# MengAiDev/SmokePhysAI

Measured on AMD Instinct MI355X. Metric: simulated+encoded frames/sec at 256^2 grid, batch 64, higher is better.
Workload: dtype f32 stencil + bf16x3 encoder (split-bf16 MFMA, fp32 accumulate)

## Files before the change

### smokephysai_amd/csrc/stencil.hip

```cpp
#include <map>
#include <mutex>

#include "stencil.h"

#include <math.h>
#include <stdlib.h>
#include <type_traits>

namespace smk {

#define TX 64
#define TY 4

__device__ __forceinline__ float clampf(float x, float lo, float hi) {
    float t = x < lo ? lo : x;
    return t > hi ? hi : t;
}
__device__ __forceinline__ int clampi(int x, int lo, int hi) {
    int t = x < lo ? lo : x;
    return t > hi ? hi : t;
}

__global__ void k_zero_state(Geom g, StateView s, const uint8_t *mask) {
    int b = blockIdx.z;
// ... 161 lines not shown
            float lap = v[(size_t)iu * g.pv + g.W] + v[(size_t)id * g.pv + g.W];
            lap = lap + vc.w;
            lap = lap + c;
            lap = lap - 4.0f * c;
            out.v[b * g.sv + (size_t)i * g.pv + g.W] = c + g.coef_uv * lap;
        }
    }
}

hipError_t launch_buoy_diffuse(const Geom &g, StateView in, StateView out, hipStream_t st) {
    if (g.W % 4 == 0 && g.pc % 4 == 0 && g.pv % 4 == 0) {
        dim3 grid(cdiv(g.W / 4, TX), cdiv(g.H + 1, TY), g.B), block(TX, TY);
        hipLaunchKernelGGL(k_buoy_diffuse4, grid, block, 0, st, g, in, out);
        return hipGetLastError();
    }
    dim3 grid(cdiv(g.W + 1, TX), cdiv(g.H + 1, TY), g.B), block(TX, TY);
    hipLaunchKernelGGL(k_buoy_diffuse, grid, block, 0, st, g, in, out);
    return hipGetLastError();
}

__global__ void k_divergence(Geom g, const float *u, const float *v, float *div, int dp, size_t ds) {
    int b = blockIdx.z;
    int j = blockIdx.x * TX + threadIdx.x, i = blockIdx.y * TY + threadIdx.y;
    if (i >= g.H || j >= g.W) return;
    const float *ub = u + b * g.su, *vb = v + b * g.sv;
    float a = ub[(size_t)(i + 1) * g.pc + j] - ub[(size_t)i * g.pc + j];
    a = a + vb[(size_t)i * g.pv + j + 1];
    a = a - vb[(size_t)i * g.pv + j];
    div[b * ds + (size_t)i * dp + j] = __fdiv_rn(a, g.dt);
}

hipError_t launch_divergence(const Geom &g, const float *u, const float *v, float *div, int dp, size_t ds,
                             hipStream_t st) {
    dim3 grid(cdiv(g.W, TX), cdiv(g.H, TY), g.B), block(TX, TY);
    hipLaunchKernelGGL(k_divergence, grid, block, 0, st, g, u, v, div, dp, ds);
    return hipGetLastError();
}

__global__ void k_jacobi_sweep(Geom g, const float *p, float *pn, const float *div) {
    int b = blockIdx.z;
    int j = blockIdx.x * TX + threadIdx.x, i = blockIdx.y * TY + threadIdx.y;
    if (i >= g.H || j >= g.W) return;
    const float *pb = p + b * g.sc;
    size_t o = (size_t)i * g.pc + j;
    float r = 0.f;
    if (i > 0 && i < g.H - 1 && j > 0 && j < g.W - 1) {
        float s = pb[o - g.pc] + pb[o + g.pc];
        s = s + pb[o - 1];
        s = s + pb[o + 1];
        s = s - div[b * g.sc + o];
        r = 0.25f * s;
    }
    pn[b * g.sc + o] = r;
}

__global__ void k_copy_cells(Geom g, const float *src, float *dst) {
    int j = blockIdx.x * TX + threadIdx.x, i = blockIdx.y * TY + threadIdx.y;
    if (i >= g.H || j >= g.W) return;
    size_t o = blockIdx.z * g.sc + (size_t)i * g.pc + j;
    dst[o] = src[o];
}

__device__ __forceinline__ float wave_shr1(float x) {
    return __builtin_bit_cast(float, __builtin_amdgcn_mov_dpp(__builtin_bit_cast(int, x), 0x138, 0xf, 0xf, true));
}
__device__ __forceinline__ float wave_shl1(float x) {
    return __builtin_bit_cast(float, __builtin_amdgcn_mov_dpp(__builtin_bit_cast(int, x), 0x130, 0xf, 0xf, true));
}

constexpr int JB_NW = 16;

template <int VEC> struct VecT;
template <> struct VecT<1> { using type = float; };
template <> struct VecT<2> { using type = float2; };
template <> struct VecT<4> { using type = float4; };
template <> struct VecT<8> { using type = float4; };
template <int VEC>
__device__ __forceinline__ void ldv(float (&dst)[VEC], const float *src) {
    using V = typename VecT<VEC>::type;
    constexpr int N = sizeof(V) / 4;
#pragma unroll
    for (int q = 0; q < VEC / N; ++q) {
        const V t = reinterpret_cast<const V *>(src)[q];
        const float *f = reinterpret_cast<const float *>(&t);
#pragma unroll
        for (int c = 0; c < N; ++c) dst[q * N + c] = f[c];
    }
}
template <int VEC>
__device__ __forceinline__ void stv(float *dst, const float (&src)[VEC]) {
    using V = typename VecT<VEC>::type;
    constexpr int N = sizeof(V) / 4;
#pragma unroll
    for (int q = 0; q < VEC / N; ++q) {
        V t;
        float *f = reinterpret_cast<float *>(&t);
#pragma unroll
        for (int c = 0; c < N; ++c) f[c] = src[q * N + c];
        reinterpret_cast<V *>(dst)[q] = t;
    }
}

struct JacobiSync {
    unsigned *flags;
    unsigned *status;
    float *x0, *x1;
    unsigned base;
    int chunks, nb, grid0, ngrids, abort_slot, fault;
    long long timeout_ticks;
    const float *u_in, *v_in, *d_in;
    float *d_out;
};

template <int VEC>
__device__ __forceinline__ void ldv_sc1(float (&dst)[VEC], __amdgpu_buffer_rsrc_t rs, unsigned byte_off) {
    typedef unsigned int u32x4 __attribute__((ext_vector_type(4)));
    typedef unsigned int u32x2 __attribute__((ext_vector_type(2)));
    if constexpr (VEC >= 4) {
#pragma unroll
        for (int q = 0; q < VEC / 4; ++q) {
            const u32x4 t = __builtin_amdgcn_raw_buffer_load_b128(rs, byte_off + 16 * q, 0, 16);
#pragma unroll
            for (int c = 0; c < 4; ++c) dst[4 * q + c] = __uint_as_float(t[c]);
        }
    } else if constexpr (VEC == 2) {
        const u32x2 t = __builtin_amdgcn_raw_buffer_load_b64(rs, byte_off, 0, 16);
        dst[0] = __uint_as_float(t[0]);
        dst[1] = __uint_as_float(t[1]);
    } else {
        dst[0] = __uint_as_float(__builtin_amdgcn_raw_buffer_load_b32(rs, byte_off, 0, 16));
    }
}
template <int VEC>
__device__ __forceinline__ void stv_sc1(__amdgpu_buffer_rsrc_t rs, unsigned byte_off, const float (&src)[VEC]) {
    typedef unsigned int u32x4 __attribute__((ext_vector_type(4)));
    typedef unsigned int u32x2 __attribute__((ext_vector_type(2)));
    if constexpr (VEC >= 4) {
#pragma unroll
        for (int q = 0; q < VEC / 4; ++q) {
            u32x4 t;
#pragma unroll
            for (int c = 0; c < 4; ++c) t[c] = __float_as_uint(src[4 * q + c]);
            __builtin_amdgcn_raw_buffer_store_b128(t, rs, byte_off + 16 * q, 0, 16);
        }
    } else if constexpr (VEC == 2) {
        u32x2 t;
        t[0] = __float_as_uint(src[0]);
        t[1] = __float_as_uint(src[1]);
        __builtin_amdgcn_raw_buffer_store_b64(t, rs, byte_off, 0, 16);
    } else {
        __builtin_amdgcn_raw_buffer_store_b32(__float_as_uint(src[0]), rs, byte_off, 0, 16);
    }
}

template <int VEC, int RPW, int MODE, bool PERSIST = false, bool FOLD = false>
__global__ __launch_bounds__(JB_NW * 64) void k_jacobi_band(Geom g, const float *__restrict__ p_in,
                                                            float *__restrict__ p_out, float *__restrict__ div,
                                                            float *__restrict__ u, float *__restrict__ v,
                                                            int iters, int BR, JacobiSync sy) {
    constexpr int TR = JB_NW * RPW, ROWF = 64 * VEC;
    __shared__ float edge[2][JB_NW][2][ROWF];
    __shared__ int handoff_failed;
    const int lane = threadIdx.x & 63, wave = threadIdx.x >> 6;
    int band_, grid_, nb_;
    if constexpr (PERSIST) {
        nb_ = sy.nb;
        const int id = blockIdx.x;
        if ((sy.ngrids & 7) == 0) {
            const int xcd = id & 7, slot = id >> 3;
            grid_ = (slot / nb_) * 8 + xcd;
            band_ = slot % nb_;
        } else {
            grid_ = id / nb_;
            band_ = id % nb_;
        }
        grid_ += sy.grid0;
    } else {
        band_ = blockIdx.x; grid_ = blockIdx.y; nb_ = gridDim.x;
    }
    const int band = band_, b = grid_, nb = nb_, halo = BR;
    const int e_rows = TR - halo, m_rows = TR - 2 * halo;
    const int own0 = band == 0 ? 0 : e_rows + (band - 1) * m_rows;
    int own1 = band == nb - 1 ? g.H : e_rows + band * m_rows;
    own1 = own1 < g.H ? own1 : g.H;
    int r0 = band == 0 ? 0 : (band == nb - 1 ? g.H - TR : own0 - halo);
    if (r0 > g.H - TR) r0 = g.H - TR;
    if (r0 < 0) r0 = 0;
    const int row0 = r0 + wave * RPW, j0 = lane * VEC;
    const size_t base = b * g.sc + (size_t)row0 * g.pc + j0;
    float pv[RPW][VEC], dv[RPW][VEC];
    const bool first_col = lane == 0, last_col = lane == 63;
    if constexpr (FOLD) {
        const float *ui = sy.u_in + b * g.su, *vi = sy.v_in + b * g.sv, *di = sy.d_in + b * g.sc;
        float *uo = u + b * g.su, *vo = v + b * g.sv, *dout = sy.d_out + b * g.sc;
        const int H = g.H, W = g.W;
        auto rowu = [&](int i, float (&x)[VEC]) {
            i = i < 0 ? 0 : (i > H ? H : i);
            ldv<VEC>(x, ui + (size_t)i * g.pc + j0);
        };
        auto rowdv = [&](int i, float (&dx)[VEC], float (&vx)[VEC], float &vW) {
            i = i < 0 ? 0 : (i > H - 1 ? H - 1 : i);
            ldv<VEC>(dx, di + (size_t)i * g.pc + j0);
            ldv<VEC>(vx, vi + (size_t)i * g.pv + j0);
            vW = vi[(size_t)i * g.pv + W];
#pragma unroll
            for (int c = 0; c < VEC; ++c) {
                const float bb = dx[c] * 0.1f;
                vx[c] = vx[c] + g.dt * bb;
            }
        };
        auto lap = [&](const float (&cc)[VEC], const float (&up)[VEC], const float (&dn)[VEC], float left, float right, float coef,
                       float (&o)[VEC]) {
#pragma unroll
            for (int c = 0; c < VEC; ++c) {
                float l = up[c] + dn[c];
                l = l + (c > 0 ? cc[c - 1] : left);
                l = l + (c < VEC - 1 ? cc[c + 1] : right);
                l = l - 4.0f * cc[c];
                o[c] = cc[c] + coef * l;
            }
        };
        float um[VEC], uc[VEC], un[VEC], dm[VEC], dc[VEC], dn[VEC], vm[VEC], vc[VEC], vn[VEC], vWm, vWc, vWn;
        rowu(row0 - 1, um);
        rowu(row0, uc);
        rowdv(row0 - 1, dm, vm, vWm);
        rowdv(row0, dc, vc, vWc);
        float u2prev[VEC], v2keep[VEC + 1];
#pragma unroll
        for (int k = 0; k <= RPW; ++k) {
            const int gi = row0 + k;
            rowu(gi + 1, un);
            float u2[VEC];
            {
                const float sl = wave_shr1(uc[VEC - 1]), sr = wave_shl1(uc[0]);
                lap(uc, um, un, first_col ? uc[0] : sl, last_col ? uc[VEC - 1] : sr, g.coef_uv, u2);
            }
            if ((gi >= own0 && gi < own1) || (gi == H && band == nb - 1)) stv<VEC>(uo + (size_t)gi * g.pc + j0, u2);
            if (k > 0) {
#pragma unroll
                for (int c = 0; c < VEC; ++c) {
                    float a = u2[c] - u2prev[c];
                    a = a + v2keep[c + 1];
                    a = a - v2keep[c];
                    dv[k - 1][c] = __fdiv_rn(a, g.dt);
                }
            }
#pragma unroll
            for (int c = 0; c < VEC; ++c) { u2prev[c] = u2[c]; um[c] = uc[c]; uc[c] = un[c]; }
            if (k < RPW) {
                rowdv(gi + 1, dn, vn, vWn);
                float d2[VEC], v2[VEC];
                {
                    const float sl = wave_shr1(dc[VEC - 1]), sr = wave_shl1(dc[0]);
                    lap(dc, dm, dn, first_col ? dc[0] : sl, last_col ? dc[VEC - 1] : sr, g.coef_d, d2);
                }
                {
                    const float sl = wave_shr1(vc[VEC - 1]), sr = wave_shl1(vc[0]);
                    lap(vc, vm, vn, first_col ? vc[0] : sl, last_col ? vWc : sr, g.coef_uv, v2);
                }
                float lw = vWm + vWn;
                lw = lw + vc[VEC - 1];
                lw = lw + vWc;
                lw = lw - 4.0f * vWc;
                const float v2W = vWc + g.coef_uv * lw;
                if (gi >= own0 && gi < own1) {
                    stv<VEC>(dout + (size_t)gi * g.pc + j0, d2);
                    stv<VEC>(vo + (size_t)gi * g.pv + j0, v2);
                    if (last_col) vo[(size_t)gi * g.pv + W] = v2W;
                }
                const float nx = wave_shl1(v2[0]);
#pragma unroll
                for (int c = 0; c < VEC; ++c) v2keep[c] = v2[c];
                v2keep[VEC] = last_col ? v2W : nx;
#pragma unroll
                for (int c = 0; c < VEC; ++c) { dm[c] = dc[c]; dc[c] = dn[c]; vm[c] = vc[c]; vc[c] = vn[c]; }
                vWm = vWc; vWc = vWn;
            }
        }
    }
#pragma unroll
    for (int k = 0; k < RPW; ++k)
#pragma unroll
        for (int c = 0; c < VEC; ++c) pv[k][c] = p_in[base + (size_t)k * g.pc + c];
    if constexpr (FOLD) {
    } else if (MODE & 1) {
        const float *ub = u + b * g.su + (size_t)row0 * g.pc + j0, *vb = v + b * g.sv + (size_t)row0 * g.pv + j0;
#pragma unroll
        for (int k = 0; k < RPW; ++k) {
            float vr[VEC + 1];
#pragma unroll
            for (int c = 0; c <= VEC; ++c) vr[c] = vb[(size_t)k * g.pv + c];
#pragma unroll
            for (int c = 0; c < VEC; ++c) {
                float a = ub[(size_t)(k + 1) * g.pc + c] - ub[(size_t)k * g.pc + c];
                a = a + vr[c + 1];
                a = a - vr[c];
                dv[k][c] = __fdiv_rn(a, g.dt);
            }
            const int gi = row0 + k;
            if (!PERSIST && gi >= own0 && gi < own1) {
#pragma unroll
                for (int c = 0; c < VEC; ++c) div[base + (size_t)k * g.pc + c] = dv[k][c];
            }
        }
    } else {
#pragma unroll
        for (int k = 0; k < RPW; ++k)
#pragma unroll
            for (int c = 0; c < VEC; ++c) dv[k][c] = div[base + (size_t)k * g.pc + c];
    }
    const int ring_k = __builtin_amdgcn_readfirstlane(row0 == 0 ? 0 : (row0 + RPW == g.H ? RPW - 1 : -1));
    auto sweep = [&](const float (&src)[RPW][VEC], float (&dst)[RPW][VEC], int par) {
#pragma unroll
        for (int c = 0; c < VEC; ++c) {
            edge[par][wave][0][j0 + c] = src[0][c];
            edge[par][wave][1][j0 + c] = src[RPW - 1][c];
        }
        __builtin_amdgcn_sched_barrier(0);
        auto row = [&](int k, const float (&up)[VEC], const float (&dn)[VEC]) {
            const float lin = wave_shr1(src[k][VEC - 1]), rin = wave_shl1(src[k][0]);
#pragma unroll
            for (int c = 0; c < VEC; ++c) {
                const float l = c > 0 ? src[k][c - 1] : lin;
                const float r = c < VEC - 1 ? src[k][c + 1] : rin;
                float sm = up[c] + dn[c];
                sm = sm + l;
                sm = sm + r;
                sm = sm - dv[k][c];
                dst[k][c] = 0.25f * sm;
            }
            dst[k][0] = first_col ? 0.f : dst[k][0];
            dst[k][VEC - 1] = last_col ? 0.f : dst[k][VEC - 1];
        };
#pragma unroll
        for (int k = 1; k < RPW - 1; ++k) row(k, src[k - 1], src[k + 1]);
        __builtin_amdgcn_sched_barrier(0);
        __syncthreads();
        const float *eu = &edge[par][wave > 0 ? wave - 1 : 0][1][j0];
        const float *ed = &edge[par][wave < JB_NW - 1 ? wave + 1 : JB_NW - 1][0][j0];
        float above[VEC], below[VEC];
#pragma unroll
        for (int c = 0; c < VEC; ++c) {
            above[c] = eu[c];
            below[c] = ed[c];
        }
        if (RPW == 1) {
            row(0, above, below);
        } else {
            row(0, above, src[1]);
            row(RPW - 1, src[RPW - 2], below);
        }
#pragma unroll
        for (int c = 0; c < VEC; ++c) {
            dst[0][c] = ring_k == 0 ? 0.f : dst[0][c];
            dst[RPW - 1][c] = ring_k == RPW - 1 ? 0.f : dst[RPW - 1][c];
        }
    };
    float pw[RPW][VEC];
    auto run = [&](int n) {
        int it = 0;
        for (; it + 2 <= n; it += 2) {
            sweep(pv, pw, 0);
            sweep(pw, pv, 1);
        }
        if (it < n) {
            sweep(pv, pw, 0);
#pragma unroll
            for (int k = 0; k < RPW; ++k)
#pragma unroll
                for (int c = 0; c < VEC; ++c) pv[k][c] = pw[k][c];
        }
    };
    if constexpr (!PERSIST) {
        run(iters);
    } else {
        const int me = b * nb + band;
        const unsigned row_off = (unsigned)(base * sizeof(float));
        const unsigned pitch_b = (unsigned)(g.pc * sizeof(float));
        const unsigned xbytes = (unsigned)((size_t)(sy.grid0 + sy.ngrids) * g.sc * sizeof(float));
        const __amdgpu_buffer_rsrc_t rx0 = __builtin_amdgcn_make_buffer_rsrc(sy.x0, 0, xbytes, 0x00020000);
        const __amdgpu_buffer_rsrc_t rx1 = __builtin_amdgcn_make_buffer_rsrc(sy.x1, 0, xbytes, 0x00020000);
        int done = 0;
        if (threadIdx.x == 0) handoff_failed = 0;
        for (int c = 0; c < sy.chunks; ++c) {
            const int n = (iters - done + (sy.chunks - c) - 1) / (sy.chunks - c);
            run(n);
            done += n;
            if (c == sy.chunks - 1) break;
            const __amdgpu_buffer_rsrc_t rx = (c & 1) ? rx1 : rx0;
#pragma unroll
            for (int k = 0; k < RPW; ++k) {
                const int gi = row0 + k;
                const bool pub = (band > 0 && gi >= own0 && gi < own0 + halo) || (band < nb - 1 && gi >= own1 - halo && gi < own1);
                if (pub) stv_sc1<VEC>(rx, row_off + k * pitch_b, pv[k]);
            }
            asm volatile("s_waitcnt vmcnt(0)" ::: "memory");
            __syncthreads();
            if (threadIdx.x == 0) {
                const unsigned tgt = sy.base + (unsigned)c + 1u;
                if (!(sy.fault && me == sy.grid0 * nb))
                    __hip_atomic_store(sy.flags + me, tgt, __ATOMIC_RELAXED, __HIP_MEMORY_SCOPE_AGENT);
                const long long t0 = wall_clock64();
                for (;;) {
                    const bool up = band == 0 ||
                        (int)(__hip_atomic_load(sy.flags + me - 1, __ATOMIC_RELAXED, __HIP_MEMORY_SCOPE_AGENT) - tgt) >= 0;
                    const bool dn = band == nb - 1 ||
                        (int)(__hip_atomic_load(sy.flags + me + 1, __ATOMIC_RELAXED, __HIP_MEMORY_SCOPE_AGENT) - tgt) >= 0;
                    if (up && dn) break;
                    if (__hip_atomic_load(sy.flags + sy.abort_slot, __ATOMIC_RELAXED, __HIP_MEMORY_SCOPE_AGENT) != 0u) {
                        handoff_failed = 1;
                        break;
                    }
                    if (wall_clock64() - t0 > sy.timeout_ticks) {
                        __hip_atomic_store(sy.flags + sy.abort_slot, 1u, __ATOMIC_RELAXED, __HIP_MEMORY_SCOPE_AGENT);
                        __hip_atomic_store(sy.status, 1u, __ATOMIC_RELAXED, __HIP_MEMORY_SCOPE_SYSTEM);
                        handoff_failed = 1;
                        break;
                    }
                    __builtin_amdgcn_s_sleep(2);
                }
            }
            __syncthreads();
#pragma unroll
            for (int k = 0; k < RPW; ++k) {
                const int gi = row0 + k;
                const bool need = (gi >= own0 - halo && gi < own0) || (gi >= own1 && gi < own1 + halo);
                if (need) ldv_sc1<VEC>(pv[k], rx, row_off + k * pitch_b);
            }
        }
        if (sy.chunks > 1 && handoff_failed) {
#pragma unroll
            for (int k = 0; k < RPW; ++k)
#pragma unroll
                for (int c = 0; c < VEC; ++c) pv[k][c] = __builtin_nanf("");
        }
    }
#pragma unroll
    for (int k = 0; k < RPW; ++k) {
        const int gi = row0 + k;
        if (gi >= own0 && gi < own1) {
#pragma unroll
            for (int c = 0; c < VEC; ++c) p_out[base + (size_t)k * g.pc + c] = pv[k][c];
        }
    }
    if (MODE & 2) {
        __syncthreads();
#pragma unroll
        for (int c = 0; c < VEC; ++c) edge[0][wave][1][j0 + c] = pv[RPW - 1][c];
        __syncthreads();
        float above[VEC];
#pragma unroll
        for (int c = 0; c < VEC; ++c) above[c] = edge[0][wave > 0 ? wave - 1 : 0][1][j0 + c];
        float *ub = u + b * g.su + (size_t)row0 * g.pc + j0, *vb = v + b * g.sv + (size_t)row0 * g.pv + j0;
#pragma unroll
        for (int k = 0; k < RPW; ++k) {
            const int gi = row0 + k;
            const float lin = wave_shr1(pv[k][VEC - 1]);
            if (gi >= own0 && gi < own1) {
                float un[VEC], vn[VEC];
                ldv<VEC>(un, ub + (size_t)k * g.pc);
                ldv<VEC>(vn, vb + (size_t)k * g.pv);
#pragma unroll
                for (int c = 0; c < VEC; ++c) {
                    if (gi >= 1) {
                        const float pu = k > 0 ? pv[k - 1][c] : above[c];
                        const float gr = pv[k][c] - pu;
                        un[c] = un[c] - g.dt * gr;
                    }
                    const float pl = c > 0 ? pv[k][c - 1] : lin;
                    const float gr = pv[k][c] - pl;
                    const float nv = vn[c] - g.dt * gr;
                    vn[c] = (c == 0 && first_col) ? vn[c] : nv;
                }
                if (gi >= 1) stv<VEC>(ub + (size_t)k * g.pc, un);
                stv<VEC>(vb + (size_t)k * g.pv, vn);
            }
        }
    }
}

struct StencilKnobs {
    bool persist, fault;
    StencilKnobs() {
        auto flag = [](const char *n, bool dflt) { const char *v = getenv(n); return v ? v[0] == '1' : dflt; };
        persist = flag("SMK_JACOBI_PERSIST", true);
        fault = flag("SMK_JACOBI_FAULT", false);
    }
};
static const StencilKnobs &knobs() {
    static const StencilKnobs k;
    return k;
}

struct JacobiPlan { int vec, rpw, br, nb, halo; };
static bool plan_jacobi(const Geom &g, JacobiPlan &pl, int iters = 100, bool persist = false) {
    if (g.W % 64 != 0 || g.W / 64 > 8 || (g.W / 64 & (g.W / 64 - 1)) || g.pc % 4 != 0) return false;
    pl.vec = g.W / 64;
    const int rpws[] = {2, 3, 4, 6, 8};
    double best = 1e30;
    bool ok = false;
    for (int rpw : rpws) {
        if (pl.vec * rpw > 32) continue;
        const int TR = JB_NW * rpw;
        if (TR > g.H) continue;
        for (int nb = 1; nb <= g.H / 8; ++nb) {
            int halo = nb == 1 ? 1 << 20 : (nb * TR - g.H) / (2 * nb - 2);
            if (nb == 1 && TR != g.H) continue;
            if (nb * TR < g.H || halo < 2) continue;
            if (nb > 1) {
                if (halo > 64) halo = 64;
                if (halo > (TR - 1) / 2) halo = (TR - 1) / 2;
                if ((TR - halo) + (nb - 2) * (TR - 2 * halo) >= g.H) continue;
            }
            if (persist && nb > 1) {
                const int e_rows = TR - halo, m_rows = TR - 2 * halo, last = g.H - (e_rows + (nb - 2) * m_rows);
                if (e_rows <= halo || last <= halo || (nb > 2 && m_rows <= halo) || nb > 64) continue;
            }
            const int br = halo;
            const double wgs = (double)nb * g.B, rounds = ceil(wgs / 256.0);
            const double cost_per_sweep = rounds * TR * (1.33 / 96.0), launch = 6.0;
            const double cost = persist ? launch + (ceil((double)iters / halo) - 1) * 3.5 + iters * cost_per_sweep
                                        : 2 * ceil(0.5 * iters / halo) * launch + iters * cost_per_sweep;
            if (cost < best) { best = cost; pl.rpw = rpw; pl.br = br; pl.nb = nb; pl.halo = halo; ok = true; }
        }
    }
    return ok;
}


template <int VEC, int MODE>
static void launch_band(const Geom &g, const JacobiPlan &pl, const float *pin, float *pout, float *div, float *u, float *v,
                        int iters, hipStream_t st) {
    dim3 grid(pl.nb, g.B), block(JB_NW * 64);
    const JacobiSync none{};
    switch (pl.rpw) {
        case 2: hipLaunchKernelGGL((k_jacobi_band<VEC, 2, MODE>), grid, block, 0, st, g, pin, pout, div, u, v, iters, pl.br, none); break;
        case 3: hipLaunchKernelGGL((k_jacobi_band<VEC, 3, MODE>), grid, block, 0, st, g, pin, pout, div, u, v, iters, pl.br, none); break;
        case 4: hipLaunchKernelGGL((k_jacobi_band<VEC, 4, MODE>), grid, block, 0, st, g, pin, pout, div, u, v, iters, pl.br, none); break;
        case 6: if constexpr (VEC <= 4) hipLaunchKernelGGL((k_jacobi_band<VEC, 6, MODE>), grid, block, 0, st, g, pin, pout, div, u, v, iters, pl.br, none); break;
        case 8: if constexpr (VEC <= 4) hipLaunchKernelGGL((k_jacobi_band<VEC, 8, MODE>), grid, block, 0, st, g, pin, pout, div, u, v, iters, pl.br, none); break;
    }
}

template <int VEC, bool FOLD>
static void launch_persist(const Geom &g, const JacobiPlan &pl, float *p, float *u, float *v, int iters, const JacobiSync &sy, hipStream_t st) {
    dim3 grid(pl.nb * sy.ngrids), block(JB_NW * 64);
    switch (pl.rpw) {
        case 2: hipLaunchKernelGGL((k_jacobi_band<VEC, 2, 3, true, FOLD>), grid, block, 0, st, g, p, p, nullptr, u, v, iters, pl.br, sy); break;
        case 3: hipLaunchKernelGGL((k_jacobi_band<VEC, 3, 3, true, FOLD>), grid, block, 0, st, g, p, p, nullptr, u, v, iters, pl.br, sy); break;
        case 4: hipLaunchKernelGGL((k_jacobi_band<VEC, 4, 3, true, FOLD>), grid, block, 0, st, g, p, p, nullptr, u, v, iters, pl.br, sy); break;
        case 6: if constexpr (VEC <= 4) hipLaunchKernelGGL((k_jacobi_band<VEC, 6, 3, true, FOLD>), grid, block, 0, st, g, p, p, nullptr, u, v, iters, pl.br, sy); break;
        case 8: if constexpr (VEC <= 4) hipLaunchKernelGGL((k_jacobi_band<VEC, 8, 3, true, FOLD>), grid, block, 0, st, g, p, p, nullptr, u, v, iters, pl.br, sy); break;
    }
}
template <bool FOLD>
static void launch_persist_vec(const Geom &g, const JacobiPlan &pl, float *p, float *u, float *v, int iters, const JacobiSync &sy, hipStream_t st) {
    switch (pl.vec) {
        case 1: launch_persist<1, FOLD>(g, pl, p, u, v, iters, sy, st); break;
        case 2: launch_persist<2, FOLD>(g, pl, p, u, v, iters, sy, st); break;
        case 4: launch_persist<4, FOLD>(g, pl, p, u, v, iters, sy, st); break;
        case 8: launch_persist<8, false>(g, pl, p, u, v, iters, sy, st); break;
    }
}

static bool persist_chunks(const Geom &g, const JacobiPlan &pl, int iters, int &chunks) {
    const int TR = JB_NW * pl.rpw;
    if (pl.nb == 1) { chunks = 1; return true; }
    if (pl.nb > 64 || (size_t)g.B * g.sc * sizeof(float) >= (1ull << 31)) return false;
    const int e_rows = TR - pl.halo, m_rows = TR - 2 * pl.halo, last = g.H - (e_rows + (pl.nb - 2) * m_rows);
    int min_owned = e_rows < last ? e_rows : last;
    if (pl.nb > 2 && m_rows < min_owned) min_owned = m_rows;
    if (min_owned < pl.halo + 1) return false;
    chunks = (iters + pl.halo - 1) / pl.halo;
    if (chunks < 2) chunks = 2;
    while ((iters + chunks - 1) / chunks > pl.halo || iters / chunks > pl.halo - 1) ++chunks;
    return chunks <= iters;
}

template <int MODE>
static void launch_band_vec(const Geom &g, const JacobiPlan &pl, const float *pin, float *pout, float *div, float *u, float *v,
                            int iters, hipStream_t st) {
    switch (pl.vec) {
        case 1: launch_band<1, MODE>(g, pl, pin, pout, div, u, v, iters, st); break;
        case 2: launch_band<2, MODE>(g, pl, pin, pout, div, u, v, iters, st); break;
        case 4: launch_band<4, MODE>(g, pl, pin, pout, div, u, v, iters, st); break;
        case 8: launch_band<8, MODE>(g, pl, pin, pout, div, u, v, iters, st); break;
    }
}

hipError_t launch_jacobi(const Geom &g, float *p, float *p2, const float *div, int iters, hipStream_t st) {
    if (iters <= 0) return hipSuccess;
    dim3 grid(cdiv(g.W, TX), cdiv(g.H, TY), g.B), block(TX, TY);
    JacobiPlan pl;
    float *cur = p, *nxt = p2;
    if (plan_jacobi(g, pl, iters)) {
        int L = 2 * ((iters + 2 * pl.halo - 1) / (2 * pl.halo));
        if (iters == 1) L = 1;
        int done = 0;
        for (int c = 0; c < L; ++c) {
            const int n = (iters - done + (L - c) - 1) / (L - c);
            launch_band_vec<0>(g, pl, cur, nxt, const_cast<float *>(div), nullptr, nullptr, n, st);
            done += n;
            float *t = cur; cur = nxt; nxt = t;
        }
    } else {
        for (int it = 0; it < iters; ++it) {
            hipLaunchKernelGGL(k_jacobi_sweep, grid, block, 0, st, g, cur, nxt, div);
            float *t = cur; cur = nxt; nxt = t;
        }
    }
    if (cur != p) hipLaunchKernelGGL(k_copy_cells, grid, block, 0, st, g, cur, p);
    return hipGetLastError();
}

hipError_t project_sync_create(ProjectSync &ps, int B) {
    ps.flags_len = B * 64 + 1;
    hipError_t e = hipMalloc((void **)&ps.flags, ps.flags_len * sizeof(unsigned));
    if (e == hipSuccess) e = hipMemset(ps.flags, 0, ps.flags_len * sizeof(unsigned));
    if (e == hipSuccess) e = hipHostMalloc((void **)&ps.status, sizeof(unsigned), hipHostMallocMapped);
    if (e == hipSuccess) *ps.status = 0u;
    return e;
}
void project_sync_destroy(ProjectSync &ps) {
    if (ps.flags) (void)hipFree(ps.flags);
    if (ps.status) (void)hipHostFree((void *)ps.status);
    ps.flags = nullptr;
    ps.status = nullptr;
}

static bool use_persist(const Geom &g, const ProjectSync *ps, int iters, JacobiPlan &pl, int &chunks) {
    if (!ps || !ps->flags || ps->disabled || !knobs().persist || iters < 2) return false;
    if (!plan_jacobi(g, pl, iters, true) || pl.halo < 3) return false;
    if (pl.nb > device_num_cu()) return false;
    return persist_chunks(g, pl, iters, chunks);
}

static std::unique_lock<std::mutex> order_persistent_launch(hipStream_t st) {
    struct Last { hipStream_t stream = nullptr; hipEvent_t ev = nullptr; bool any = false; };
    static std::mutex mu;
    static std::map<int, Last> last;
    int dev = 0;
    (void)hipGetDevice(&dev);
    std::unique_lock<std::mutex> lk(mu);
    Last &l = last[dev];
    if (l.any && l.stream != st) {
        if (!l.ev) (void)hipEventCreateWithFlags(&l.ev, hipEventDisableTiming);
        if (l.ev && hipEventRecord(l.ev, l.stream) == hipSuccess) (void)hipStreamWaitEvent(st, l.ev, 0);
        else (void)hipGetLastError();
    }
    l.stream = st;
    l.any = true;
    return lk;
}

bool project_sync_take_timeout(ProjectSync &ps) {
    if (!ps.status || *ps.status == 0u) return false;
    *ps.status = 0u;
    ps.disabled = true;
    return true;
}

hipError_t launch_project(const Geom &g, float *u, float *v, float *p, float *p2, float *div, int iters, hipStream_t st, ProjectSync *ps,
                          const StateView *fold_in, float *fold_d_out, bool *folded) {
    JacobiPlan pl;
    if (folded) *folded = false;
    if (ps && project_sync_take_timeout(*ps)) {
        return hipErrorLaunchTimeOut;
    }
    int chunks = 0;
    hipStreamCaptureStatus cap_status = hipStreamCaptureStatusNone;
    const bool capturing = hipStreamIsCapturing(st, &cap_status) == hipSuccess && cap_status != hipStreamCaptureStatusNone;
    if (!capturing && use_persist(g, ps, iters, pl, chunks)) {
        int per = device_num_cu() / pl.nb;
        if (per >= 8) per &= ~7;
        JacobiSync sy{};
        sy.flags = ps->flags; sy.status = const_cast<unsigned *>(ps->status); sy.x0 = div; sy.x1 = p2;
        sy.base = ps->seq; sy.chunks = chunks; sy.nb = pl.nb; sy.abort_slot = ps->flags_len - 1; sy.fault = knobs().fault ? 1 : 0;
        sy.timeout_ticks = knobs().fault ? 200000ll : 50000000ll;
        ps->seq += (unsigned)chunks;
        const std::unique_lock<std::mutex> launch_order = order_persistent_launch(st);
        const bool fold = fold_in && fold_d_out && pl.vec <= 4 && g.pv % 4 == 0 && g.pc % 4 == 0;
        if (fold) {
            sy.u_in = fold_in->u; sy.v_in = fold_in->v; sy.d_in = fold_in->d; sy.d_out = fold_d_out;
            if (folded) *folded = true;
        }
        for (int g0 = 0; g0 < g.B; g0 += per) {
            sy.grid0 = g0;
            sy.ngrids = g.B - g0 < per ? g.B - g0 : per;
            if (fold) launch_persist_vec<true>(g, pl, p, u, v, iters, sy, st);
            else launch_persist_vec<false>(g, pl, p, u, v, iters, sy, st);
        }
        return hipGetLastError();
    }
    if (iters < 2 || !plan_jacobi(g, pl, iters) || pl.halo < 3) {
        hipError_t e = launch_divergence(g, u, v, div, g.pc, g.sc, st);
        if (e != hipSuccess) return e;
        e = launch_jacobi(g, p, p2, div, iters, st);
        if (e != hipSuccess) return e;
        return launch_grad_subtract(g, u, v, p, st);
    }
    const int cap = pl.halo - 1;
    const int L = 2 * ((iters + 2 * cap - 1) / (2 * cap));
    float *cur = p, *nxt = p2;
    int done = 0;
    for (int c = 0; c < L; ++c) {
        const int n = (iters - done + (L - c) - 1) / (L - c);
        if (c == 0) launch_band_vec<1>(g, pl, cur, nxt, div, u, v, n, st);
        else if (c == L - 1) launch_band_vec<2>(g, pl, cur, nxt, div, u, v, n, st);
        else launch_band_vec<0>(g, pl, cur, nxt, div, u, v, n, st);
        done += n;
        float *t = cur; cur = nxt; nxt = t;
    }
    return hipGetLastError();
}

hipError_t launch_buoy_project(const Geom &g, StateView in, StateView out, float *p, float *div, int iters, hipStream_t st, ProjectSync *ps) {
    bool folded = false;
    JacobiPlan pl;
    int chunks = 0;
    hipStreamCaptureStatus cs = hipStreamCaptureStatusNone;
    const bool capturing = hipStreamIsCapturing(st, &cs) == hipSuccess && cs != hipStreamCaptureStatusNone;
    const bool pending_error = ps && ps->status && *ps->status != 0u;
    if (!capturing && !pending_error && use_persist(g, ps, iters, pl, chunks) && pl.vec <= 4 && g.pv % 4 == 0 && g.pc % 4 == 0) {
        const hipError_t e = launch_project(g, out.u, out.v, p, out.p, div, iters, st, ps, &in, out.d, &folded);
        if (e != hipSuccess || folded) return e;
        return hipErrorUnknown;
    }
    hipError_t e = launch_buoy_diffuse(g, in, out, st);
    if (e != hipSuccess) return e;
    return launch_project(g, out.u, out.v, p, out.p, div, iters, st, ps);
}

std::string describe_projection(const Geom &g, int iters, const ProjectSync *ps) {
    JacobiPlan pl;
    char buf[1280];
    int chunks = 0;
    const bool persist = use_persist(g, ps, iters, pl, chunks);
    if (!persist && (iters < 2 || !plan_jacobi(g, pl, iters) || pl.halo < 3)) {
        snprintf(buf, sizeof buf, "{\"kernel\": \"k_jacobi_sweep\", \"launches\": %d, \"sweeps\": %d, \"bound\": \"hbm (one pass over p and div per sweep)\"}",
                 iters + 2, iters);
        return buf;
    }
    const int cap = pl.halo - 1, TR = JB_NW * pl.rpw;
    const int per = persist ? (device_num_cu() / pl.nb >= 8 ? (device_num_cu() / pl.nb) & ~7 : device_num_cu() / pl.nb) : 0;
    const int L = persist ? (g.B + per - 1) / per : 2 * ((iters + 2 * cap - 1) / (2 * cap));
    const int parts = persist ? chunks : L;
    const double wgs = (double)pl.nb * g.B, rounds = ceil(wgs / device_num_cu());
    const double valu_us_per_sweep = rounds * (TR / 4.0) * 18.0 * 2.6 / 2100.0;
    snprintf(buf, sizeof buf,
             "{\"kernel\": \"k_jacobi_band<%d,%d>\", \"persistent\": %s, \"bands_per_grid\": %d, \"rows_per_workgroup\": %d, \"halo_rows\": %d, "
             "\"workgroups\": %d, \"launches\": %d, \"halo_handoffs\": %d, \"sweeps\": %d, \"sweeps_per_chunk\": %d, \"redundant_row_factor\": %.3f, "
             "\"vector_issue_us_per_sweep_estimate\": %.3f, \"vector_issue_us_total_estimate\": %.1f, "
             "\"bound\": \"on-chip: sweeps x (vector issue of rows_per_workgroup rows + one LDS publish/barrier/read round trip); p and div are "
             "register-resident %s\"}",
             pl.vec, pl.rpw, persist ? "true" : "false", pl.nb, TR, pl.halo, (int)wgs, L, persist ? chunks - 1 : 0, iters, (iters + parts - 1) / parts,
             (double)pl.nb * TR / g.H, valu_us_per_sweep, valu_us_per_sweep * iters,
             persist ? "for the whole projection; bands hand halo rows to their neighbours through HBM between chunks" : "within a launch");
    return buf;
}

__global__ void k_grad_subtract(Geom g, float *u, float *v, const float *p) {
    int b = blockIdx.z;
    int j = blockIdx.x * TX + threadIdx.x, i = blockIdx.y * TY + threadIdx.y;
    const float *pb = p + b * g.sc;
    if (i >= 1 && i < g.H && j < g.W) {
        float *c = u + b * g.su + (size_t)i * g.pc + j;
        float gr = pb[(size_t)i * g.pc + j] - pb[(size_t)(i - 1) * g.pc + j];
        *c = *c - g.dt * gr;
    }
    if (i < g.H && j >= 1 && j < g.W) {
        float *c = v + b * g.sv + (size_t)i * g.pv + j;
        float gr = pb[(size_t)i * g.pc + j] - pb[(size_t)i * g.pc + j - 1];
        *c = *c - g.dt * gr;
    }
}

hipError_t launch_grad_subtract(const Geom &g, float *u, float *v, const float *p, hipStream_t st) {
    dim3 grid(cdiv(g.W, TX), cdiv(g.H, TY), g.B), block(TX, TY);
    hipLaunchKernelGGL(k_grad_subtract, grid, block, 0, st, g, u, v, p);
    return hipGetLastError();
}

__device__ __forceinline__ float bilinear(const float *f, int h, int w, int pitch, float y, float x, int *ox0, int *oy0) {
    int x0 = (int)floorf(x), y0 = (int)floorf(y);
    int x1 = x0 + 1, y1 = y0 + 1;
    x0 = clampi(x0, 0, w - 1); x1 = clampi(x1, 0, w - 1);
    y0 = clampi(y0, 0, h - 1); y1 = clampi(y1, 0, h - 1);
    float fx0 = (float)x0, fx1 = (float)x1, fy0 = (float)y0, fy1 = (float)y1;
    float wa = (fx1 - x) * (fy1 - y);
    float wb = (x - fx0) * (fy1 - y);
    float wc = (fx1 - x) * (y - fy0);
    float wd = (x - fx0) * (y - fy0);
    float r = wa * f[(size_t)y0 * pitch + x0] + wb * f[(size_t)y0 * pitch + x1];
    r = r + wc * f[(size_t)y1 * pitch + x0];
    r = r + wd * f[(size_t)y1 * pitch + x1];
    if (ox0) { *ox0 = x0; *oy0 = y0; }
    return r;
}

template <int KIND>
__global__ void k_advect(Geom g, const float *field, float *out, const float *u, const float *v, float *frames,
                         int64_t fsb, const float *fractal, float fint, int32_t *x0o, int32_t *y0o) {
    constexpr bool IS_U = KIND == 0, IS_V = KIND == 1;
    const int R = IS_U ? g.H + 1 : g.H, C = IS_V ? g.W + 1 : g.W;
    const int pitch = IS_V ? g.pv : g.pc;
    const size_t fs = IS_U ? g.su : (IS_V ? g.sv : g.sc);
    int b = blockIdx.z;
    int j = blockIdx.x * TX + threadIdx.x, i = blockIdx.y * TY + threadIdx.y;
    if (i >= R || j >= C) return;
    const float *ub = u + b * g.su, *vb = v + b * g.sv, *fb = field + b * fs;
    float Y = (float)i, X = (float)j;
    float xu = clampf(X + 0.5f, 0.f, (float)(g.W - 1));
    float ui = bilinear(ub, g.H + 1, g.W, g.pc, Y, xu, nullptr, nullptr);
    float yv = clampf(Y + 0.5f, 0.f, (float)(g.H - 1));
    float vi = bilinear(vb, g.H, g.W + 1, g.pv, yv, X, nullptr, nullptr);
    float px = clampf(X - g.dt * ui, 0.f, (float)(C - 1));
    float py = clampf(Y - g.dt * vi, 0.f, (float)(R - 1));
    int x0, y0;
    float r = bilinear(fb, R, C, pitch, py, px, &x0, &y0);
    if (x0o) {
        size_t o = ((size_t)b * R + i) * C + j;
        x0o[o] = x0; y0o[o] = y0;
    }
    if (KIND == 2) {
        r = r * 0.995f;
        if (frames) {
            float fr = r;
            if (fractal) {
                float t = fint * fractal[(size_t)i * g.W + j];
                t = t * r;
                fr = r + t;
            }
            frames[(size_t)b * fsb + (size_t)i * g.W + j] = fr;
        }
    }
    if (out) out[b * fs + (size_t)i * pitch + j] = r;
}

hipError_t launch_advect(const Geom &g, int kind, const float *field, float *out, const float *u, const float *v,
                         float *frames, int64_t fsb, const float *fractal, float fint, int32_t *x0, int32_t *y0,
                         hipStream_t st) {
    dim3 block(TX, TY);
    if (kind == 0) {
        dim3 grid(cdiv(g.W, TX), cdiv(g.H + 1, TY), g.B);
        hipLaunchKernelGGL(k_advect<0>, grid, block, 0, st, g, field, out, u, v, frames, fsb, fractal, fint, x0, y0);
    } else if (kind == 1) {
        dim3 grid(cdiv(g.W + 1, TX), cdiv(g.H, TY), g.B);
        hipLaunchKernelGGL(k_advect<1>, grid, block, 0, st, g, field, out, u, v, frames, fsb, fractal, fint, x0, y0);
    } else if (kind == 3) {
        dim3 grid(cdiv(g.W, TX), cdiv(g.H, TY), g.B);
        hipLaunchKernelGGL(k_advect<3>, grid, block, 0, st, g, field, out, u, v, frames, fsb, fractal, fint, x0, y0);
    } else {
        dim3 grid(cdiv(g.W, TX), cdiv(g.H, TY), g.B);
        hipLaunchKernelGGL(k_advect<2>, grid, block, 0, st, g, field, out, u, v, frames, fsb, fractal, fint, x0, y0);
    }
    return hipGetLastError();
}


__device__ __attribute__((noinline)) float far_value2(const float *f, int pitch, int Rf, int Cf, float dt, int y, int x, float ui, float vi) {
    const float px = clampf((float)x - dt * ui, 0.f, (float)(Cf - 1));
    const float py = clampf((float)y - dt * vi, 0.f, (float)(Rf - 1));
    const int x0 = (int)px, y0 = (int)py;
    int x1 = x0 + 1, y1 = y0 + 1;
    x1 = x1 > Cf - 1 ? Cf - 1 : x1;
    y1 = y1 > Rf - 1 ? Rf - 1 : y1;
    const float fx0 = (float)x0, fx1 = (float)x1, fy0 = (float)y0, fy1 = (float)y1;
    const float wa = (fx1 - px) * (fy1 - py);
    const float wb = (px - fx0) * (fy1 - py);
    const float wc = (fx1 - px) * (py - fy0);
    const float wd = (px - fx0) * (py - fy0);
    float r = wa * f[(size_t)y0 * pitch + x0] + wb * f[(size_t)y0 * pitch + x1];
    r = r + wc * f[(size_t)y1 * pitch + x0];
    r = r + wd * f[(size_t)y1 * pitch + x1];
    return r;
}


template <int R, int NW, int BU>
__global__ __launch_bounds__(NW * 64) void k_advect_rows(Geom g, StateView in, StateView out, float *frames, int64_t fsb,
                                                         const float *__restrict__ fractal, float fint) {
    constexpr int TYR = R * NW, TXC = 64, NT = NW * 64;
    constexpr int WR = TYR + 3, WC = TXC + 3, WP = 68, WPL = WR * WP;
    constexpr int NST = (WR * WC + NT - 1) / NT;
    __shared__ float U2s[WPL], V2s[WPL], D2s[WPL];
    const int H = g.H, W = g.W, pc = g.pc, pv = g.pv;
    const int ntx = (W + TXC - 1) / TXC, nty = (H + TYR - 1) / TYR;
    unsigned tile = xcd_contiguous(blockIdx.x, gridDim.x);
    const int tix = tile % ntx; tile /= ntx;
    const int tiy = tile % nty;
    const int b = tile / nty;
    const int x0 = tix * TXC, y0 = tiy * TYR;
    const int tid = threadIdx.x, lane = tid & 63, wv = __builtin_amdgcn_readfirstlane(tid >> 6);
    const float *u2 = in.u + b * g.su, *v2 = in.v + b * g.sv, *d2 = in.d + b * g.sc;
    float *uo = out.u + b * g.su, *vo = out.v + b * g.sv, *dn = out.d + b * g.sc;
    float *fr = frames ? frames + (size_t)b * fsb : nullptr;
    const float dt = g.dt;

    {
        float ru[NST], rv[NST], rd[NST];
#pragma unroll
        for (int it = 0; it < NST; ++it) {
            const int e0 = tid + it * NT, e = e0 < WR * WC ? e0 : WR * WC - 1;
            const int r = e / WC, c = e - r * WC;
            const int gy = y0 - 1 + r, gx = x0 - 1 + c;
            const int yc = clampi(gy, 0, H - 1), xc = clampi(gx, 0, W - 1);
            ru[it] = u2[(unsigned)(clampi(gy, 0, H) * pc + xc)];
            rv[it] = v2[(unsigned)(yc * pv + clampi(gx, 0, W))];
            rd[it] = d2[(unsigned)(yc * pc + xc)];
// ... 294 lines not shown
```

Before: 211,000.

## Pipeline LDS edge-row exchange across Jacobi sweeps and retune band cost model

Each sweep now computes a wave's two edge rows first, using neighbour rows fetched during the previous sweep. It then publishes them to LDS and runs the interior rows around the barrier, so the LDS stores and the neighbour read are hidden behind vector work. The pipelined order is skipped for the persistent VEC=4, RPW=8 variant, presumably to stay under the register cap. The planner's cost model is also retuned: per-sweep cost now scales with vector width, and handoff chunks are counted explicitly. The retune can select a different band configuration, and the pipelined path holds extra registers (the above/below rows) live across the sweep.

```diff
diff --git a/smokephysai_amd/csrc/stencil.hip b/smokephysai_amd/csrc/stencil.hip
--- a/smokephysai_amd/csrc/stencil.hip
+++ b/smokephysai_amd/csrc/stencil.hip
@@ -337,6 +337,9 @@
         __builtin_amdgcn_raw_buffer_store_b32(__float_as_uint(src[0]), rs, byte_off, 0, 16);
     }
 }
+
+constexpr bool jb_pipelined(int vec, int rpw, bool persist) { return !(persist && vec == 4 && rpw == 8); }
+constexpr int jb_rows_before_barrier(int rpw) { return rpw > 2 ? 1 : 0; }
 
 template <int VEC, int RPW, int MODE, bool PERSIST = false, bool FOLD = false>
 __global__ __launch_bounds__(JB_NW * 64) void k_jacobi_band(Geom g, const float *__restrict__ p_in,
@@ -495,54 +498,82 @@
             for (int c = 0; c < VEC; ++c) dv[k][c] = div[base + (size_t)k * g.pc + c];
     }
     const int ring_k = __builtin_amdgcn_readfirstlane(row0 == 0 ? 0 : (row0 + RPW == g.H ? RPW - 1 : -1));
-    auto sweep = [&](const float (&src)[RPW][VEC], float (&dst)[RPW][VEC], int par) {
+    static_assert(RPW >= 2, "the sweep keeps a wave's first and last row apart");
+    auto row = [&](const float (&src)[RPW][VEC], float (&dst)[RPW][VEC], int k, const float (&up)[VEC], const float (&dn)[VEC]) {
+        const float lin = wave_shr1(src[k][VEC - 1]), rin = wave_shl1(src[k][0]);
 #pragma unroll
         for (int c = 0; c < VEC; ++c) {
-            edge[par][wave][0][j0 + c] = src[0][c];
-            edge[par][wave][1][j0 + c] = src[RPW - 1][c];
-        }
-        __builtin_amdgcn_sched_barrier(0);
-        auto row = [&](int k, const float (&up)[VEC], const float (&dn)[VEC]) {
-            const float lin = wave_shr1(src[k][VEC - 1]), rin = wave_shl1(src[k][0]);
-#pragma unroll
-            for (int c = 0; c < VEC; ++c) {
-                const float l = c > 0 ? src[k][c - 1] : lin;
-                const float r = c < VEC - 1 ? src[k][c + 1] : rin;
-                float sm = up[c] + dn[c];
-                sm = sm + l;
-                sm = sm + r;
-                sm = sm - dv[k][c];
-                dst[k][c] = 0.25f * sm;
-            }
-            dst[k][0] = first_col ? 0.f : dst[k][0];
-            dst[k][VEC - 1] = last_col ? 0.f : dst[k][VEC - 1];
-        };
-#pragma unroll
-        for (int k = 1; k < RPW - 1; ++k) row(k, src[k - 1], src[k + 1]);
-        __builtin_amdgcn_sched_barrier(0);
-        __syncthreads();
+            const float l = c > 0 ? src[k][c - 1] : lin;
+            const float r = c < VEC - 1 ? src[k][c + 1] : rin;
+            float sm = up[c] + dn[c];
+            sm = sm + l;
+            sm = sm + r;
+            sm = sm - dv[k][c];
+            dst[k][c] = 0.25f * sm;
+        }
+        dst[k][0] = first_col ? 0.f : dst[k][0];
+        dst[k][VEC - 1] = last_col ? 0.f : dst[k][VEC - 1];
+    };
+    auto publish = [&](const float (&r)[RPW][VEC], int par) {
+#pragma unroll
+        for (int c = 0; c < VEC; ++c) {
+            edge[par][wave][0][j0 + c] = r[0][c];
+            edge[par][wave][1][j0 + c] = r[RPW - 1][c];
+        }
+    };
+    float above[VEC], below[VEC];
+    auto fetch = [&](int par) {
         const float *eu = &edge[par][wave > 0 ? wave - 1 : 0][1][j0];
         const float *ed = &edge[par][wave < JB_NW - 1 ? wave + 1 : JB_NW - 1][0][j0];
-        float above[VEC], below[VEC];
 #pragma unroll
         for (int c = 0; c < VEC; ++c) {
             above[c] = eu[c];
             below[c] = ed[c];
         }
-        if (RPW == 1) {
-            row(0, above, below);
-        } else {
-            row(0, above, src[1]);
-            row(RPW - 1, src[RPW - 2], below);
-        }
+    };
+    auto edge_rows = [&](const float (&src)[RPW][VEC], float (&dst)[RPW][VEC]) {
+        row(src, dst, 0, above, src[1]);
+        row(src, dst, RPW - 1, src[RPW - 2], below);
 #pragma unroll
         for (int c = 0; c < VEC; ++c) {
             dst[0][c] = ring_k == 0 ? 0.f : dst[0][c];
             dst[RPW - 1][c] = ring_k == RPW - 1 ? 0.f : dst[RPW - 1][c];
         }
     };
+    constexpr bool PIPE = jb_pipelined(VEC, RPW, PERSIST);
+    constexpr int NA = jb_rows_before_barrier(RPW);
+    auto sweep = [&](const float (&src)[RPW][VEC], float (&dst)[RPW][VEC], int par) {
+        if constexpr (PIPE) {
+            edge_rows(src, dst);
+            publish(dst, par);
+            __builtin_amdgcn_sched_barrier(0);
+#pragma unroll
+            for (int k = 1; k < 1 + NA; ++k) row(src, dst, k, src[k - 1], src[k + 1]);
+            __builtin_amdgcn_sched_barrier(0);
+            __syncthreads();
+            fetch(par);
+            __builtin_amdgcn_sched_barrier(0);
+#pragma unroll
+            for (int k = 1 + NA; k < RPW - 1; ++k) row(src, dst, k, src[k - 1], src[k + 1]);
+            __builtin_amdgcn_sched_barrier(0);
+        } else {
+            publish(src, par);
+            __builtin_amdgcn_sched_barrier(0);
+#pragma unroll
+            for (int k = 1; k < RPW - 1; ++k) row(src, dst, k, src[k - 1], src[k + 1]);
+            __builtin_amdgcn_sched_barrier(0);
+            __syncthreads();
+            fetch(par);
+            edge_rows(src, dst);
+        }
+    };
     float pw[RPW][VEC];
     auto run = [&](int n) {
+        if constexpr (PIPE) {
+            publish(pv, 1);
+            __syncthreads();
+            fetch(1);
+        }
         int it = 0;
         for (; it + 2 <= n; it += 2) {
             sweep(pv, pw, 0);
@@ -703,8 +734,14 @@
             }
             const int br = halo;
             const double wgs = (double)nb * g.B, rounds = ceil(wgs / 256.0);
-            const double cost_per_sweep = rounds * TR * (1.33 / 96.0), launch = 6.0;
-            const double cost = persist ? launch + (ceil((double)iters / halo) - 1) * 3.5 + iters * cost_per_sweep
+            const double cost_per_sweep = rounds * TR * ((0.15 + 0.17 * pl.vec) / 96.0), launch = 6.0, handoff = 2.8, fixed_sweeps = 13.0;
+            int chunks = 1;
+            if (persist && nb > 1) {
+                chunks = (iters + halo - 1) / halo;
+                if (chunks < 2) chunks = 2;
+                while (chunks < iters && ((iters + chunks - 1) / chunks > halo || iters / chunks > halo - 1)) ++chunks;
+            }
+            const double cost = persist ? launch + (chunks - 1) * handoff + (iters + fixed_sweeps) * cost_per_sweep
                                         : 2 * ceil(0.5 * iters / halo) * launch + iters * cost_per_sweep;
             if (cost < best) { best = cost; pl.rpw = rpw; pl.br = br; pl.nb = nb; pl.halo = halo; ok = true; }
         }
@@ -918,7 +955,7 @@
 
 std::string describe_projection(const Geom &g, int iters, const ProjectSync *ps) {
     JacobiPlan pl;
-    char buf[1280];
+    char buf[1792];
     int chunks = 0;
     const bool persist = use_persist(g, ps, iters, pl, chunks);
     if (!persist && (iters < 2 || !plan_jacobi(g, pl, iters) || pl.halo < 3)) {
@@ -936,10 +973,14 @@
              "{\"kernel\": \"k_jacobi_band<%d,%d>\", \"persistent\": %s, \"bands_per_grid\": %d, \"rows_per_workgroup\": %d, \"halo_rows\": %d, "
              "\"workgroups\": %d, \"launches\": %d, \"halo_handoffs\": %d, \"sweeps\": %d, \"sweeps_per_chunk\": %d, \"redundant_row_factor\": %.3f, "
              "\"vector_issue_us_per_sweep_estimate\": %.3f, \"vector_issue_us_total_estimate\": %.1f, "
-             "\"bound\": \"on-chip: sweeps x (vector issue of rows_per_workgroup rows + one LDS publish/barrier/read round trip); p and div are "
+             "\"bound\": \"on-chip: sweeps x vector issue of rows_per_workgroup rows, one barrier per sweep (%s); p and div are "
              "register-resident %s\"}",
              pl.vec, pl.rpw, persist ? "true" : "false", pl.nb, TR, pl.halo, (int)wgs, L, persist ? chunks - 1 : 0, iters, (iters + parts - 1) / parts,
              (double)pl.nb * TR / g.H, valu_us_per_sweep, valu_us_per_sweep * iters,
+             jb_pipelined(pl.vec, pl.rpw, persist)
+                 ? "the LDS edge-row exchange is pipelined over two sweeps: a wave's two edge rows and their publish come first, the interior rows "
+                   "cover the stores and the read of the next sweep's neighbour rows"
+                 : "plain order at the register cap: publish, interior rows, barrier, read of the neighbour rows, the two edge rows",
              persist ? "for the whole projection; bands hand halo rows to their neighbours through HBM between chunks" : "within a launch");
     return buf;
 }
```

After: 216,600 (median of 6 runs). +2.6%, better.
